# antbern/gridmap-slam-robot

Hardware: AMD Instinct MI355X
Metric: particle-scan evals/sec (higher is better)
Workload: dtype f64; 1 GPU; C3: 16384 particles/GPU x 720 beams (697 hits), 2048x2048 grid @ 0.02 m, full scan step (score+normalise+resample+ray-cast+likelihood rebuild; the rebuild is dirty-tile / factor-table-only: bit-identical results, likelihoodData on demand -- the reference's own every-cell rebuild is cpu_baseline.gpu_like_for_like_ms_per_step); particles_total=16384, particles_per_gpu=16384, beams=720, maps=1, maps_total=1, parallelism=single GPU, inputs=resident in HBM

## Files before the change

gridmap_slam_robot_amd/csrc/gms_fused_kernels.hip:

```cpp
#include "gms_map_kernels.hip"
#include "gms_pf_kernels.hip"
#include "gms_slam_kernels.hip"

#ifndef GMS_APPLY_BLOCKS_RIDING
#define GMS_APPLY_BLOCKS_RIDING 512
#endif

#ifndef RCF_RAYS
#define RCF_RAYS 4
#endif

template <bool LOGNORM>
__global__ void __launch_bounds__(256)
k_norm_raycast(const gms_beam *__restrict__ beams, const double *__restrict__ partials, int64_t nblk_global, int32_t B,
               int32_t nw_max, uint32_t n_ray_blocks, uint32_t n_norm_blocks, uint32_t n_near_blocks, int32_t n,
               double *__restrict__ w, const float *__restrict__ pose, int64_t offset, uint32_t *__restrict__ cnt,
               int32_t *__restrict__ bbox, PackedParticle *__restrict__ packed, double *__restrict__ cum,
               double *__restrict__ chunk_tot, int64_t nchunks, double *__restrict__ p2, PfStatsDev *__restrict__ stats,
               double *__restrict__ logd, uint32_t *__restrict__ cnt_pend, const int32_t *__restrict__ bbox_pend,
               const double *__restrict__ logw_lognorm, uint32_t *__restrict__ res_ticket, double *__restrict__ res_pre, GridDev g) {
    extern __shared__ __align__(16) unsigned char smem[];
    GMS_STAMP(GMS_STAMP_ROW(2, blockIdx.x), 0);
    if (blockIdx.x >= n_ray_blocks + n_norm_blocks) {
        apply_body(g, logd, cnt_pend, bbox_pend, nullptr, blockIdx.x - n_ray_blocks - n_norm_blocks, 0,
                   gridDim.x - n_ray_blocks - n_norm_blocks);
        GMS_STAMP(GMS_STAMP_ROW(2, blockIdx.x), 15);
        return;
    }
    if (blockIdx.x < n_ray_blocks) {
        __shared__ RedLds L;
        const bool near = blockIdx.x >= n_ray_blocks - n_near_blocks;
        const RayPre pre = near ? raycast_near_prologue(beams, B, B, blockIdx.x - (n_ray_blocks - n_near_blocks), 0, smem)
                                : raycast_prologue<RCF_RAYS, 4>(beams, B, B, nullptr, nw_max, blockIdx.x, 0, smem);
        const int cols[4] = { COL_SUM, COL_XW, COL_YW, COL_TW };
        double f[4];
        if (LOGNORM) {
            fold_lognorm<4>(partials, nblk_global, cols, f, L);
        } else {
            fold_sums<4>(partials, nblk_global, cols, f, L);
        }
        const float wpose[3] = { (float)(f[1] / f[0]), (float)(f[2] / f[0]), (float)(f[3] / f[0]) };
        GMS_STAMP(GMS_STAMP_ROW(2, blockIdx.x), 1);
        if (near) raycast_near_body(g, pre, wpose, cnt, bbox, 0, smem);
        else raycast_body<false, RCF_RAYS, 4>(g, pre, wpose, B, nullptr, cnt, bbox, nullptr, nullptr, 0, nullptr, blockIdx.x, 0, smem, n_near_blocks ? 1 : 0);
    } else {
        normalize_pack_body(partials, nblk_global, w, pose, n, offset, packed, cum, chunk_tot, nchunks, p2, stats,
                            blockIdx.x - n_ray_blocks, 0, LOGNORM ? logw_lognorm : (const double *)nullptr, res_ticket, n_norm_blocks,
                            res_pre, smem);
        GMS_STAMP(GMS_STAMP_ROW(2, blockIdx.x), 14);
    }
}

__global__ void __launch_bounds__(256)
k_partials_apply(const double *__restrict__ part, const float *__restrict__ pose, PfStatsDev *__restrict__ lognorm_stats, int32_t n,
                 int32_t part_nseg, int64_t offset, int64_t nblk_global, double *__restrict__ w, double *__restrict__ logw,
                 double *__restrict__ partials, double *__restrict__ logd, uint32_t *__restrict__ cnt,
                 const int32_t *__restrict__ bbox, int32_t *__restrict__ bbox_idle, GridDev g) {
    if (blockIdx.x < (uint32_t)nblk_global)
        partials_body(w, logw, pose, n, offset, nblk_global, partials, part, part_nseg, blockIdx.x, blockIdx.y, lognorm_stats);
    else
        apply_body(g, logd, cnt, bbox, bbox_idle, blockIdx.x - (uint32_t)nblk_global, blockIdx.y, gridDim.x - (uint32_t)nblk_global);
}

__global__ void __launch_bounds__(256)
k_partials_pack_apply(const double *__restrict__ part, const float *__restrict__ pose, int32_t n, int32_t part_nseg,
                      uint32_t n_local_blocks, int64_t offset, int64_t nblk_global, double *__restrict__ w, double *__restrict__ logw,
                      double *__restrict__ partials, PackedParticle *__restrict__ packed_local, double *__restrict__ logd,
                      uint32_t *__restrict__ cnt, const int32_t *__restrict__ bbox, int32_t *__restrict__ bbox_idle, GridDev g) {
    if (blockIdx.x < n_local_blocks) {
// ... 58 lines not shown
        likelihood_body<KH, SPLIT>(g, logd, lik, fac, fac_stride, taps_g, bbox, 1, tiles_x, tiles_y, blockIdx.x - n_res_blocks,
                                   blockIdx.y, gridDim.x - n_res_blocks, smem, cnt_pending, tile_state, lik_mode);
    GMS_STAMP(GMS_STAMP_ROW(3, blockIdx.x), blockIdx.x < n_res_blocks ? 1 : 2);
}

__global__ void __launch_bounds__(256)
k_deskew_motion(const double *__restrict__ angle, const double *__restrict__ distance, const uint8_t *__restrict__ hit, int32_t length,
                double d_center, double d_theta, gms_beam *__restrict__ beams_out, uint32_t n_deskew_blocks,
                float *__restrict__ pose, float *__restrict__ cs, int32_t n, int64_t offset, double d_center_sd, double d_theta_sd,
                uint64_t seed, uint64_t sequence) {
    if (blockIdx.x < n_deskew_blocks)
        deskew_body(angle, distance, hit, length, d_center, d_theta, beams_out, (int32_t)(blockIdx.x * 256u + threadIdx.x));
    else
        motion_body(pose, cs, n, offset, d_center, d_theta, d_center_sd, d_theta_sd, seed, sequence, 0,
                    (int32_t)((blockIdx.x - n_deskew_blocks) * 256u + threadIdx.x));
}

bool gms_can_pair_launches(const gms_pf *pf, int32_t B) {
    const gms_map *m = pf->map;
    return pf->n_maps == 1 && B > 0 && B <= GMS_MAX_BEAMS && !m->need_full_build && m->pair_launches;
}

void gms_launch_norm_raycast(gms_pf *pf, const double *d_partials, PackedParticle *d_packed_local, bool own,
                             const gms_beam *d_beams, int32_t B) {
    gms_map *m = pf->map;
    ProfScope ps(m, GMS_K_RAYCAST);
    const uint32_t n_near = rc_near_blocks(m, B);
    const uint32_t n_ray = (uint32_t)((B + RCF_RAYS - 1) / RCF_RAYS) + n_near, n_norm = (uint32_t)((pf->n + 255) / 256);
    const int64_t nch = nchunks_of(pf);
    const size_t smem_pre = own ? (size_t)(nch + 1 + (nch + 63) / 64 + 1) * sizeof(double) : 0;
    size_t smem = rc_smem(m, RCF_RAYS, n_near);
    if (smem < smem_pre) smem = smem_pre;
    const uint32_t n_apply = m->apply_pending ? apply_blocks(m, GMS_APPLY_BLOCKS_RIDING) : 0u;
    int32_t *pend = map_box(m);
    int32_t *bb = n_apply ? map_box(m, true) : pend;
    auto launch = [&](auto lognorm) {
        gms_launch<k_norm_raycast<lognorm()>>(m, dim3(n_ray + n_norm + n_apply), dim3(256), smem, d_beams, d_partials, nblk_global_of(pf), B,
                                              rc_nw_max(m), n_ray, n_norm, n_near, pf->n, pf->d_w, pf->d_pose, pf->offset, m->d_cnt, bb, d_packed_local,
                                              own ? pf->d_cum : (double *)nullptr, own ? pf->d_chunk_tot : (double *)nullptr, nchunks_of(pf),
                                              own ? pf->d_p2 : (double *)nullptr, pf->d_stats, m->d_log, m->d_cnt_pend, pend,
                                              lognorm() ? (const double *)pf->d_logw : (const double *)nullptr,
                                              own ? pf->d_res_ticket : (uint32_t *)nullptr, pf->d_res_pre, m->gd);
    };
    if (gms_pf_lognorm_now(pf)) launch(gms_c<true>{}); else launch(gms_c<false>{});
    if (n_apply) gms_apply_done(m);
    pf_normalized(pf, own, own);
}

void gms_launch_partials_apply(gms_pf *pf, double *d_partials, bool apply_rides_later) {
    gms_map *m = pf->map;
    if (!m->apply_pending || apply_rides_later) { gms_launch_pf_partials(pf, d_partials); return; }
    ProfScope ps(m, GMS_K_REDUCE);
    const int64_t nblk = nblk_global_of(pf);
    const uint32_t n_apply = apply_blocks(m, GMS_APPLY_BLOCKS);
    PfStatsDev *lognorm_stats = gms_pf_lognorm_now(pf) ? pf->d_stats : (PfStatsDev *)nullptr;
    hipLaunchKernelGGL(k_partials_apply, dim3((uint32_t)nblk + n_apply, pf->n_maps), dim3(256), 0, m->stream,
                       pf->pending_nseg ? (const double *)pf->d_part : (const double *)nullptr, pf->d_pose, lognorm_stats, pf->n,
                       pf->pending_nseg, pf->offset, nblk, pf->d_w, pf->d_logw, d_partials, m->d_log, m->d_cnt_pend,
                       map_box(m), map_box(m, true), m->gd);
    pf_weights_combined(pf);
    gms_apply_done(m);
}

void gms_launch_lik_resample(gms_pf *pf, double fraction) {
    gms_map *m = pf->map;
    gms_launch_pf_chunk_sums(pf);
    const double *pre = pf->res_pre_ready ? (const double *)pf->d_res_pre : (const double *)nullptr;
// ... 68 lines not shown
```

gridmap_slam_robot_amd/csrc/gms_host.hip:

```cpp
#include <math.h>
#include <dlfcn.h>
#include <stdarg.h>
#include <stddef.h>
#include <stdio.h>
#include <stdlib.h>
#include <string.h>

#include <new>
#include <algorithm>
#include <vector>

#include "gms_internal.h"

static thread_local char g_err[512] = "";

int gms_fail(int code, const char *fmt, ...) {
    va_list ap;
    va_start(ap, fmt);
    vsnprintf(g_err, sizeof(g_err), fmt, ap);
    va_end(ap);
    return code;
}

static int32_t j_d2i_host(double d) {
// ... 829 lines not shown
    HIPCHK(hipSetDevice(m->device));
    return gms_set_stamp_buffer(m, dev_buffer) ? GMS_OK : gms_fail(GMS_ERR_STATE, "this build carries no stage stamps (compile with -DGMS_STAMPS)");
}

int gms_debug_f32(gms_map *m, int32_t op, const float *in, float *out, int64_t n) {
    REQUIRE(m && in && out && n > 0 && op >= 0 && op <= 5 && (op != 3 || n % 64 == 0), "gms_debug_f32: bad arguments");
    HIPCHK(hipSetDevice(m->device));
    float *d_a = nullptr, *d_o = nullptr;
    HIPCHK(hipMalloc(&d_a, n * sizeof(float)));
    HIPCHK(hipMalloc(&d_o, n * sizeof(float)));
    HIPCHK(hipMemcpyAsync(d_a, in, n * sizeof(float), hipMemcpyHostToDevice, m->stream));
    gms_launch_debug_f32(m, op, d_a, d_o, n);
    HIPCHK(hipMemcpyAsync(out, d_o, n * sizeof(float), hipMemcpyDeviceToHost, m->stream));
    HIPCHK(hipStreamSynchronize(m->stream));
    hipFree(d_a); hipFree(d_o);
    return GMS_OK;
}

static int64_t nblk_of(int64_t n) { return (n + GMS_BLOCK - 1) / GMS_BLOCK; }
static int64_t nchunks_of(int64_t n) { return (n + 63) / 64; }

static void pf_free_global(gms_pf *pf) {
    hipFree(pf->d_partials); hipFree(pf->d_p2); hipFree(pf->d_global_own); hipFree(pf->d_chunk_tot); hipFree(pf->d_cum);
    hipFree(pf->d_res_pre); hipFree(pf->d_res_ticket);
    pf->d_partials = pf->d_p2 = nullptr; pf->d_global = pf->d_global_own = nullptr; pf->d_chunk_tot = pf->d_cum = nullptr;
    pf->d_res_pre = nullptr; pf->d_res_ticket = nullptr; pf->res_pre_ready = 0; pf->have_global = 0;
}

static int pf_alloc_global(gms_pf *pf) {
    pf_free_global(pf);
    const size_t M = pf->n_maps;
    const size_t nblk = nblk_of(pf->n_global), nch = nchunks_of(pf->n_global);
    HIPCHK(hipMalloc(&pf->d_partials, M * nblk * GMS_PARTIAL_STRIDE * sizeof(double)));
    HIPCHK(hipMalloc(&pf->d_p2, M * nblk * 2 * sizeof(double)));
    HIPCHK(hipMalloc(&pf->d_global_own, M * pf->n_global * sizeof(PackedParticle)));
    pf->d_global = pf->d_global_own;
    HIPCHK(hipMalloc(&pf->d_chunk_tot, M * (nch + 1 + nch * 8) * sizeof(double)));
    HIPCHK(hipMalloc(&pf->d_cum, M * pf->n_global * sizeof(double)));
    HIPCHK(hipMalloc(&pf->d_res_pre, M * (nch + 3) * sizeof(double)));
    HIPCHK(hipMalloc(&pf->d_res_ticket, M * sizeof(uint32_t)));
    HIPCHK(hipMemsetAsync(pf->d_res_ticket, 0, M * sizeof(uint32_t), pf->map->stream));
    return GMS_OK;
}

int gms_pf_destroy(gms_pf *pf) {
    if (!pf) return GMS_OK;
    hipSetDevice(pf->map->device);
    hipStreamSynchronize(pf->map->stream);
    pf->map->n_filters--;
    hipFree(pf->d_pose); hipFree(pf->d_pose2); hipFree(pf->d_part); hipFree(pf->d_cs2);
    hipFree(pf->d_w); hipFree(pf->d_w2); hipFree(pf->d_logw); hipFree(pf->d_cs); hipFree(pf->d_hitbeams);
    hipFree(pf->d_nhit); hipFree(pf->d_stats); hipFree(pf->d_r01); hipFree(pf->d_idx);
    hipFree(pf->d_ord); hipFree(pf->d_perm);
    hipFree(pf->modes.d_part); hipFree(pf->modes.d_bins); hipFree(pf->modes.d_table); hipFree(pf->modes.d_ctl);
    if (pf->modes.h_ctl) hipHostFree(pf->modes.h_ctl);
    hipFree(pf->beam.d_tab); ring_free(pf->beam.ring);
// ... 382 lines not shown
                        double resample_fraction, int32_t integrate) {
    return slam_update_impl(pf, dev_xytheta, nullptr, dev_beams, B, B, r01, resample_fraction, integrate);
}

int gms_slam_update_u_dev(gms_pf *pf, double d_center, double d_theta, uint64_t seed, uint64_t sequence, const gms_beam *dev_beams,
                          int32_t B, const double *r01, double resample_fraction, int32_t integrate) {
    MotionModel mo;
    mo.d_center = d_center; mo.d_theta = d_theta; mo.seed = seed; mo.sequence = sequence;
    return slam_update_impl(pf, nullptr, &mo, dev_beams, B, B, r01, resample_fraction, integrate);
}

static int slam_update_impl(gms_pf *pf, const float *dev_xytheta, const MotionModel *motion, const gms_beam *dev_beams, int32_t B,
                            int32_t beam_stride, const double *r01, double resample_fraction, int32_t integrate) {
    REQUIRE(pf && dev_beams && r01, "null argument");
    int rc = refuse_owned_maps(pf);
    if (rc) return rc;
    gms_map *m = pf->map;
    if (pf_is_shard(pf))
        return gms_fail(GMS_ERR_STATE, "sharded filter: the collectives belong to the caller (see distributed.py)");
    const ScanIn at_pose = dev_scan(dev_beams, B, beam_stride, nullptr, pf, 0);
    rc = set_poses_and_score_dev(pf, dev_xytheta, dev_beams, B, beam_stride, pf->refine != 0, motion);
    const bool pair = !rc && integrate && !pf->reference_order && beam_stride == B;
    if (pair && gms_can_pair_launches(pf, B)) {
        gms_launch_partials_apply(pf, pf->d_partials, true);
        gms_launch_norm_raycast(pf, pf->d_partials, pf->d_global_own, true, dev_beams, B);
        return paired_likelihood_resample(pf, r01, resample_fraction);
    }
    if (pair && pf->n_maps > 1 && B > 0 && !m->need_full_build && m->pair_launches) {
        const bool ride = gms_raycast_tiled(m, B);
        gms_launch_partials_apply(pf, pf->d_partials, ride);
        gms_launch_pf_apply_partials(pf, pf->d_partials, pf->d_global_own, true);
        ScanDev d;
        scan_pose(m, at_pose, &d);
        gms_launch_raycast(m, dev_beams, B, B, d.poses, d.pose_stride, ride);
        return paired_likelihood_resample(pf, r01, resample_fraction);
    }
    if (!rc) rc = gms_pf_normalize(pf, nullptr);
    if (!rc && resample_fraction >= 0.0) rc = gms_pf_resample_if(pf, r01, resample_fraction);
    if (!rc && integrate) rc = map_scan(m, at_pose, SCAN_UPDATE_MAY_DEFER);
    return rc;
}

int gms_slam_frame(gms_pf *pf, const double *angle, const double *distance, const uint8_t *hit, int32_t length, double d_center,
                   double d_theta, uint64_t seed, uint64_t sequence, const double *r01, double resample_fraction, int32_t integrate) {
    REQUIRE(pf && angle && distance && hit && r01, "null argument");
    gms_map *m = pf->map;
    if (pf->n_maps != 1) return gms_fail(GMS_ERR_STATE, "gms_slam_frame: one map per handle (a frame is one robot's revolution)");
    if (pf_is_shard(pf))
// ... 509 lines not shown
```

gridmap_slam_robot_amd/csrc/gms_internal.h:

```cpp
#pragma once

#include <hip/hip_runtime.h>
#include <stdint.h>

#include <atomic>
#include <mutex>
#include <type_traits>
#include <vector>

#include "gridmapslam.h"

struct GridDev {
    int32_t W, H;
    int64_t cells;
    double posx, posy;
    double res;
    double rinv;
    float resf;
    double l_free, l_occ;
    int32_t extra;
    float half_tol;
    double z_hit;
    double c_rand;
    double inv_max;
// ... 176 lines not shown
    m->fac_current = 1;
    m->need_full_build = 0;
}
static inline void map_box_consumed(gms_map *m) {
    if (m->bbox_dirty) { m->bbox_cur = 1 - m->bbox_cur; m->bbox_dirty = 0; }
}

struct gms_pf {
    gms_map *map;
    int32_t n;
    int64_t offset;
    int64_t n_global;
    int32_t n_maps;
    float *d_pose;
    float *d_pose2;
    float *d_cs2;
    double *d_w, *d_w2;
    double *d_logw, *d_logw2;
    float *d_cs;
    double *d_hitbeams;
    double *d_part;
    int32_t *d_nhit;
    double *d_partials;
    double *d_p2;
    PackedParticle *d_global_own;
    double *d_chunk_tot;
    double *d_cum;
    double *d_res_pre;
    uint32_t *d_res_ticket;
    PfStatsDev *d_stats;
    PfStatsDev *h_stats;
    double *d_r01;
    const double *d_r01_src;
    double r01_scalar;
    int32_t *d_idx;
    float *h_stage;
    StageRing pose_ring;
    StageRing r01_ring;
    int32_t refine;
    float4 *d_ord;
    int32_t *d_perm;
    int32_t log_norm;
    int32_t score_threads;
    int32_t reference_order;
    int32_t score_spread;
    int32_t order_mode;
// ... 308 lines not shown
    void fetch(void *dst, size_t part, size_t bytes) { out[n_out].dst = dst; out[n_out].part = part; out[n_out++].bytes = bytes; }
    int finish(int32_t *shown);
};
struct QuerySource {
    gms_map *m;
    gms_slam *s;
    int32_t index, filter;
};
static inline QuerySource query_map(gms_map *m, int32_t mi) { return {m, nullptr, mi, 0}; }
static inline QuerySource query_slam(gms_slam *s, int32_t which) { return {s ? s->map : nullptr, s, which, 0}; }
int query_check(QuerySource &src, const char *what, const char *filter_name);
int query_plane(const QuerySource &src, int32_t mode, int32_t *d_shown, uint32_t *d_dst, const uint32_t **plane);
int gms_clear_launch(gms_map *m, const uint32_t *d_plane, const gms_clearance *c, uint16_t *d_out);
int gms_reach_inflate(gms_map *m, const uint32_t *d_obstacles, int32_t inflate, int32_t mode, const uint32_t **d_blocked);

void gms_launch_pf_init(gms_pf *pf);
void gms_launch_pf_pose_trig(gms_pf *pf, const float *d_src);
void gms_launch_pf_combine(gms_pf *pf);
void gms_launch_pf_motion(gms_pf *pf, double d_center, double d_theta, uint64_t seed, uint64_t sequence);
void gms_launch_pf_chunk_sums(gms_pf *pf);
void gms_launch_partials_apply(gms_pf *pf, double *d_partials, bool apply_rides_later = false);
bool gms_can_pair_launches(const gms_pf *pf, int32_t B);
void gms_launch_norm_raycast(gms_pf *pf, const double *d_partials, PackedParticle *d_packed_local, bool own,
                             const gms_beam *d_beams, int32_t B);
void gms_launch_lik_resample(gms_pf *pf, double fraction);
void gms_launch_deskew_motion(gms_pf *pf, const double *d_angle, const double *d_distance, const uint8_t *d_hit, int32_t length,
                              double d_center, double d_theta, uint64_t seed, uint64_t sequence);
void gms_launch_partials_pack_apply(gms_pf *pf, bool apply_rides_later = false);
void gms_launch_raycast_norm_chunks(gms_pf *pf, const gms_beam *d_beams, int32_t B, bool raycast);
void gms_launch_pf_fold_neff(gms_pf *pf);
struct MotionModel {
    double d_center, d_theta;
    uint64_t seed, sequence;
};
static inline void motion_deviations(double d_center, double d_theta, double *d_center_sd, double *d_theta_sd) {
    *d_center_sd = (0.01 + fabs(d_center) * 0.05) / 2;
    *d_theta_sd = 5 * (3.141592653589793 / 180.0) + 0.1 * fabs(d_theta);
}
void gms_launch_pf_score(gms_pf *pf, const gms_beam *d_beams, int32_t B, int32_t beam_stride, const float *d_pose_src = nullptr,
                         const MotionModel *motion = nullptr);
void gms_launch_pf_partials(gms_pf *pf, double *d_partials);
bool gms_pf_lognorm_now(const gms_pf *pf);
void gms_launch_pf_pack(gms_pf *pf, PackedParticle *d_packed);
void gms_launch_pf_apply_partials(gms_pf *pf, const double *d_partials, PackedParticle *d_packed_local, bool own);
void gms_launch_pf_stats_only(gms_pf *pf, const double *d_partials, PfStatsDev *d_stats_out);
void gms_launch_pf_resample(gms_pf *pf, double fraction );
void gms_launch_pf_refine(gms_pf *pf, const gms_beam *d_beams, int32_t B, int32_t beam_stride);
void gms_launch_pf_normalize_seq(gms_pf *pf, PfStatsDev *d_stats_out, bool normalise);
void gms_launch_pf_resample_seq(gms_pf *pf, double fraction);
SlamBufs gms_slam_bufs(const gms_slam *s);
void gms_launch_slam_likelihood(gms_map *m, const SlamBufs &sb, int32_t n);
void gms_launch_slam_deskew(gms_map *m, const double *angle, const double *distance, const uint8_t *hit, int32_t L, int32_t S, int32_t Lmax,
                            int32_t length, double d_center, double d_theta, const SlamFilterArgs *tab_src, SlamFilterArgs *tab_dst, gms_beam *d_out,
                            int32_t out_pitch);
void gms_launch_slam_particle(gms_pf *pf, const gms_beam *d_beams, int32_t B, const SlamBufs &sb, bool field_in_memory, const MotionModel *motion,
                              int32_t integrate, int64_t code_words, const SlamBatch *batch = nullptr);
void gms_launch_slam_likelihood_codes(gms_map *m, const SlamBufs &sb, int64_t code_words, int32_t n, int32_t plane);
void gms_launch_slam_codes_from_log(gms_map *m, const SlamBufs &sb, int32_t first, int32_t count, int64_t code_words);
int64_t gms_slam_code_words(int64_t cells);
void gms_launch_slam_trace(gms_pf *pf, const gms_beam *d_beams, int32_t B, int32_t particle, int32_t *d_cells, uint8_t *d_cls, int32_t cap, int32_t *d_counts);
bool gms_launch_slam_refine(gms_pf *pf, const gms_beam *d_beams, int32_t B, const SlamBufs &sb, const MotionModel *motion, int32_t field_in_lds,
                            int64_t code_words, const SlamBatch *batch = nullptr);
bool gms_slam_refine_from_planes(const gms_map *m, int32_t B, int32_t field_in_lds, int64_t code_words);
int gms_align_check_for(const gms_align_params *p, const char *who);
bool gms_slam_align_from_planes(const gms_slam *s, int32_t B);
// ... 42 lines not shown
```

gridmap_slam_robot_amd/csrc/gms_pf_kernels.hip:

```cpp
#include "gms_device.h"
#include "gms_slam_device.h"

#define SCAN_CHUNK 64
#define RES_SUB_MAX_CHUNKS 1024

__global__ void k_pf_init(float *pose, float *cs, double *w, double *logw, int64_t total, double w0) {
    int64_t i = (int64_t)blockIdx.x * blockDim.x + threadIdx.x;
    if (i < total) {
        pose[3 * i] = 0.0f; pose[3 * i + 1] = 0.0f; pose[3 * i + 2] = 0.0f;
        cs[2 * i] = 1.0f; cs[2 * i + 1] = 0.0f;
        w[i] = w0; logw[i] = 0.0;
    }
}

__global__ void __launch_bounds__(256)
k_pose_trig(const float *__restrict__ src, float *__restrict__ dst, float *__restrict__ cs, int64_t total) {
    const int64_t i = (int64_t)blockIdx.x * blockDim.x + threadIdx.x;
    if (i >= total) return;
    const float x = src[3 * i], y = src[3 * i + 1], th = src[3 * i + 2];
    dst[3 * i] = x; dst[3 * i + 1] = y; dst[3 * i + 2] = th;
    float c, s;
    pose_trig(th, c, s);
    cs[2 * i] = c; cs[2 * i + 1] = s;
}
// ... 425 lines not shown
    const int32_t wave = threadIdx.x >> 6, g4 = (wave >> 2) << 2;
    GMS_STAMP(GMS_STAMP_ROW(1, blockIdx.x), 3);
    __syncthreads();
    if ((threadIdx.x & 63) == 0) {
#pragma unroll
        for (int c = 0; c < 6; c++) L.m[c][wave] = sums[c];
        L.m[6][wave] = mv; L.m[7][wave] = mx; L.m[8][wave] = ml;
    }
    __syncthreads();
    GMS_STAMP(GMS_STAMP_ROW(1, blockIdx.x), 4);
#pragma unroll
    for (int c = 0; c < 6; c++) sums[c] = ((L.m[c][g4] + L.m[c][g4 + 1]) + L.m[c][g4 + 2]) + L.m[c][g4 + 3];
    mv = L.m[6][g4]; mx = L.m[7][g4]; ml = L.m[8][g4];
    for (int k = 1; k < 4; k++) {
        argmax_merge(mv, mx, L.m[6][g4 + k], L.m[7][g4 + k]);
        if (L.m[8][g4 + k] > ml) ml = L.m[8][g4 + k];
    }
    (void)mli;
    out[COL_SUM] = sums[0]; out[COL_NZ] = sums[1]; out[COL_SQ] = sums[2];
    out[COL_XW] = sums[3]; out[COL_YW] = sums[4]; out[COL_TW] = sums[5];
    out[COL_MAX] = mv; out[COL_ARG] = mx; out[COL_MLW] = ml;
}

__device__ __forceinline__ double fold_sum(const double *__restrict__ p, int64_t nblk, int col, double *lds) {
    double acc = 0.0;
    for (int64_t b = threadIdx.x & (GRP - 1); b < nblk; b += GRP) acc += p[b * GMS_PARTIAL_STRIDE + col];
    return group_sum(acc, lds);
}

template <int NC>
__device__ __forceinline__ void fold_sums(const double *__restrict__ p, int64_t nblk, const int (&col)[NC], double (&out)[NC],
                                          RedLds &L) {
    static_assert(NC <= GMS_PARTIAL_STRIDE, "RedLds::m has GMS_PARTIAL_STRIDE rows");
    double acc[NC];
#pragma unroll
    for (int c = 0; c < NC; c++) acc[c] = 0.0;
    for (int64_t b = threadIdx.x & (GRP - 1); b < nblk; b += GRP) {
        double v[NC];
#pragma unroll
        for (int c = 0; c < NC; c++) v[c] = p[b * GMS_PARTIAL_STRIDE + col[c]];
#pragma unroll
        for (int c = 0; c < NC; c++) acc[c] += v[c];
    }
#pragma unroll
    for (int c = 0; c < NC; c++) acc[c] = wave_sum_f64(acc[c]);
    const int32_t wave = threadIdx.x >> 6, g4 = (wave >> 2) << 2;
    __syncthreads();
    if ((threadIdx.x & 63) == 0) {
#pragma unroll
        for (int c = 0; c < NC; c++) L.m[c][wave] = acc[c];
    }
    __syncthreads();
#pragma unroll
    for (int c = 0; c < NC; c++) out[c] = ((L.m[c][g4] + L.m[c][g4 + 1]) + L.m[c][g4 + 2]) + L.m[c][g4 + 3];
}

template <int NC>
__device__ __forceinline__ void fold_sums_scaled(const double *__restrict__ p, int64_t nblk, const int (&col)[NC], double (&out)[NC],
                                                 RedLds &L, double M) {
    static_assert(NC <= GMS_PARTIAL_STRIDE, "RedLds::m has GMS_PARTIAL_STRIDE rows");
    const double R = lognorm_ref(M);
    double acc[NC];
#pragma unroll
    for (int c = 0; c < NC; c++) acc[c] = 0.0;
    for (int64_t b = threadIdx.x & (GRP - 1); b < nblk; b += GRP) {
        double v[NC];
#pragma unroll
        for (int c = 0; c < NC; c++) v[c] = p[b * GMS_PARTIAL_STRIDE + col[c]];
        const double sc = exp(lognorm_ref(p[b * GMS_PARTIAL_STRIDE + COL_MLW]) - R);
#pragma unroll
        for (int c = 0; c < NC; c++) acc[c] += v[c] * sc;
    }
#pragma unroll
    for (int c = 0; c < NC; c++) acc[c] = wave_sum_f64(acc[c]);
    const int32_t wave = threadIdx.x >> 6, g4 = (wave >> 2) << 2;
    __syncthreads();
    if ((threadIdx.x & 63) == 0) {
#pragma unroll
        for (int c = 0; c < NC; c++) L.m[c][wave] = acc[c];
    }
    __syncthreads();
#pragma unroll
    for (int c = 0; c < NC; c++) out[c] = ((L.m[c][g4] + L.m[c][g4 + 1]) + L.m[c][g4 + 2]) + L.m[c][g4 + 3];
}

__device__ __forceinline__ void fold_argmax(const double *__restrict__ p, int64_t nblk, int colv, int coli, double &mv,
                                            double &mx, RedLds &L);
template <int NC>
__device__ __forceinline__ double fold_lognorm(const double *__restrict__ p, int64_t nblk, const int (&col)[NC], double (&out)[NC], RedLds &L) {
    if (nblk > GRP) {
        double ml, mli;
        fold_argmax(p, nblk, COL_MLW, -1, ml, mli, L);
        fold_sums_scaled<NC>(p, nblk, col, out, L, ml);
        return ml;
    }
    const int64_t b = threadIdx.x & (GRP - 1);
    const bool in = b < nblk;
    double v[NC];
#pragma unroll
    for (int c = 0; c < NC; c++) v[c] = in ? p[b * GMS_PARTIAL_STRIDE + col[c]] : 0.0;
    const double mb = in ? p[b * GMS_PARTIAL_STRIDE + COL_MLW] : -INFINITY;
    double mloc = mb == mb ? mb : -INFINITY;
#define GMS_STEP_(O) { const double v2 = wave_xor<O>(mloc); if (v2 > mloc) mloc = v2; }
    GMS_BUTTERFLY(GMS_STEP_)
#undef GMS_STEP_
    const int32_t wave = threadIdx.x >> 6, g4 = (wave >> 2) << 2;
    __syncthreads();
    if ((threadIdx.x & 63) == 0) L.b[wave] = mloc;
    __syncthreads();
    double M = L.b[g4];
    for (int k = 1; k < 4; k++) if (L.b[g4 + k] > M) M = L.b[g4 + k];
    const double sc = in ? exp(lognorm_ref(mb) - lognorm_ref(M)) : 0.0;
    double acc[NC];
#pragma unroll
    for (int c = 0; c < NC; c++) acc[c] = wave_sum_f64(0.0 + v[c] * sc);
    if ((threadIdx.x & 63) == 0) {
#pragma unroll
        for (int c = 0; c < NC; c++) L.m[c][wave] = acc[c];
    }
    __syncthreads();
#pragma unroll
    for (int c = 0; c < NC; c++) out[c] = ((L.m[c][g4] + L.m[c][g4 + 1]) + L.m[c][g4 + 2]) + L.m[c][g4 + 3];
    return M;
}

__device__ __forceinline__ void fold_argmax(const double *__restrict__ p, int64_t nblk, int colv, int coli, double &mv,
                                            double &mx, RedLds &L) {
    mv = -INFINITY; mx = 9.0e15;
    bool first = true;
    for (int64_t b = threadIdx.x & (GRP - 1); b < nblk; b += GRP) {
        const double v2 = p[b * GMS_PARTIAL_STRIDE + colv], i2 = coli >= 0 ? p[b * GMS_PARTIAL_STRIDE + coli] : (double)b;
        if (first) { mv = v2; mx = i2; first = false; } else argmax_merge(mv, mx, v2, i2);
    }
    group_argmax(mv, mx, L.a, L.b);
}

__device__ __forceinline__ double fold_stats(const double *__restrict__ p, int64_t nblk, PfStatsDev *s, bool write,
                                             const float *__restrict__ pose, int64_t pose_base, int64_t pose_n, RedLds &L,
                                             const PackedParticle *__restrict__ glob = nullptr, bool lognorm = false, double *ref_out = nullptr) {
    double ml = 0.0, mli;
    if (!write) {
        if (!lognorm) return fold_sum(p, nblk, COL_SUM, L.a);
        const int c1[1] = { COL_SUM };
        double f1[1];
        ml = fold_lognorm<1>(p, nblk, c1, f1, L);
        if (ref_out) *ref_out = ml;
        return f1[0];
    }
    const int cols[5] = { COL_SUM, COL_NZ, COL_XW, COL_YW, COL_TW };
    double f[5];
    if (lognorm) { ml = fold_lognorm<5>(p, nblk, cols, f, L); if (ref_out) *ref_out = ml; }
    else fold_sums<5>(p, nblk, cols, f, L);
    const double sum = f[0], nz = f[1], xw = f[2], yw = f[3], tw = f[4];
    double mv, mx;
    fold_argmax(p, nblk, COL_MAX, COL_ARG, mv, mx, L);
    if (!lognorm) fold_argmax(p, nblk, COL_MLW, -1, ml, mli, L);
    if (threadIdx.x == 0) {
        s->n_ambiguous = 0;
        s->weight_sum = sum;
        s->max_w = lognorm ? exp(ml - lognorm_ref(ml)) : mv;
        s->strongest = mx < 8.0e15 ? (int32_t)mx : 0;
        if (!lognorm) s->n_zero = (int32_t)nz;
        s->max_logw = ml;
        s->xs = xw; s->ys = yw; s->ts = tw;
        s->wpose[0] = (float)(xw / sum);
        s->wpose[1] = (float)(yw / sum);
        s->wpose[2] = (float)(tw / sum);
        const int64_t st = (int64_t)s->strongest - pose_base;
        if (glob) {
            const PackedParticle pp = glob[s->strongest];
            s->spose[0] = pp.x; s->spose[1] = pp.y; s->spose[2] = pp.theta;
        } else if (pose && st >= 0 && st < pose_n) {
            s->spose[0] = pose[3 * st]; s->spose[1] = pose[3 * st + 1]; s->spose[2] = pose[3 * st + 2];
        }
    }
    return sum;
}

__device__ __forceinline__ int64_t block_count(int64_t n, int64_t blk) {
// ... 32 lines not shown
    const int64_t nlb = ((int64_t)n + GMS_BLOCK - 1) / GMS_BLOCK;
    double *p = partials + ((size_t)mi * nblk_global + gb) * GMS_PARTIAL_STRIDE;
    if (lb < 0 || lb >= nlb) {
        if (threadIdx.x < GMS_PARTIAL_STRIDE) p[threadIdx.x] = 0.0;
        return;
    }
    double out[GMS_PARTIAL_STRIDE];
    const size_t o = (size_t)mi * n + lb * GMS_BLOCK;
    block_partials(w + o, logw + o, pose + 3 * o, block_count(n, lb), offset + lb * GMS_BLOCK, out, L, part, mi, n,
                   part_nseg, lb * GMS_BLOCK, lognorm_stats != nullptr);
    if (threadIdx.x == 0)
        for (int k = 0; k < GMS_PARTIAL_STRIDE; k++) p[k] = out[k];
}

__global__ void __launch_bounds__(256)
k_partials(const double *__restrict__ part, const float *__restrict__ pose, PfStatsDev *__restrict__ lognorm_stats, int32_t n,
           int32_t part_nseg, int64_t offset, int64_t nblk_global, double *__restrict__ w, double *__restrict__ logw,
           double *__restrict__ partials) {
    GMS_STAMP(GMS_STAMP_ROW(1, blockIdx.x), 0);
    partials_body(w, logw, pose, n, offset, nblk_global, partials, part, part_nseg, blockIdx.x, blockIdx.y, lognorm_stats);
    GMS_STAMP(GMS_STAMP_ROW(1, blockIdx.x), 1);
}

__device__ __forceinline__ double *chunk_sub_of(double *chunk_tot_all, int64_t nchunks, int32_t n_maps, int32_t mi) {
    return chunk_tot_all + (size_t)n_maps * (nchunks + 1) + (size_t)mi * nchunks * 8;
}
__device__ __forceinline__ void block_chunk_scan(double v, int64_t i, int64_t n_pop, int64_t blk, int64_t nchunks,
                                                 double *__restrict__ cum, double *__restrict__ chunk_tot,
                                                 double *__restrict__ p2_blk, double *__restrict__ sub, bool through = false) {
    __shared__ double s_ct[4][2];
    const int32_t lane = threadIdx.x & 63, wave = threadIdx.x >> 6;
    double inc = v;
#pragma unroll
    for (int o = 1; o < 64; o <<= 1) {
        const double up = __shfl_up(inc, o, GMS_WAVE);
        if (lane >= o) inc += up;
    }
    const double sq = wave_sum_f64(v * v);
    const double tot = __shfl(inc, 63, GMS_WAVE);
    if (i < n_pop) cum[i] = inc;
    if ((lane & 7) == 7 && blk * 4 + wave < nchunks) sub[(blk * 4 + wave) * 8 + (lane >> 3)] = inc;
    if (lane == 0) {
        const int64_t c = blk * 4 + wave;
        if (c < nchunks) { if (through) store_through(&chunk_tot[c], tot); else chunk_tot[c] = tot; }
        s_ct[wave][0] = tot; s_ct[wave][1] = sq;
    }
// ... 66 lines not shown
    double tv[8];
#pragma unroll
    for (int k = 0; k < 8; k++) { const int64_t c = (int64_t)threadIdx.x + k * (int64_t)blockDim.x; tv[k] = c < nchunks ? load_coherent<true>(&tot[c]) : 0.0; }
    double norm_sum, sq_sum;
    fold_neff<true>(p2, nblk, norm_sum, sq_sum, lds);
#pragma unroll
    for (int k = 0; k < 8; k++) { const int64_t c = (int64_t)threadIdx.x + k * (int64_t)blockDim.x; if (c < nchunks) off[c] = tv[k]; }
    for (int64_t c0 = (int64_t)threadIdx.x + 8 * (int64_t)blockDim.x; c0 < nchunks; c0 += 8 * (int64_t)blockDim.x) {
        double v[8];
#pragma unroll
        for (int k = 0; k < 8; k++) { const int64_t c = c0 + k * (int64_t)blockDim.x; v[k] = c < nchunks ? load_coherent<true>(&tot[c]) : 0.0; }
#pragma unroll
        for (int k = 0; k < 8; k++) { const int64_t c = c0 + k * (int64_t)blockDim.x; if (c < nchunks) off[c] = v[k]; }
    }
    chunk_offsets_scan(off, nchunks);
    for (int64_t c = threadIdx.x; c <= nchunks; c += blockDim.x) pre[c] = off[c];
    if (threadIdx.x == 0) {
        pre[nchunks + 1] = norm_sum; pre[nchunks + 2] = sq_sum;
        stats->norm_sum = norm_sum; stats->sq_sum = sq_sum;
    }
    GMS_STAMP(GMS_STAMP_ROW(2, blockIdx.x), 13);
}

__device__ __forceinline__ void
normalize_pack_body(const double *__restrict__ partials_all, int64_t nblk_global, double *__restrict__ w,
                    const float *__restrict__ pose, int32_t n, int64_t offset, PackedParticle *__restrict__ packed,
                    double *__restrict__ cum, double *__restrict__ chunk_tot, int64_t nchunks,
                    double *__restrict__ p2_all, PfStatsDev *__restrict__ stats, uint32_t bx, uint32_t by,
                    const double *__restrict__ logw_lognorm = nullptr, uint32_t *__restrict__ ticket = nullptr,
                    uint32_t n_blocks = 0, double *__restrict__ pre = nullptr, unsigned char *smem = nullptr) {
    __shared__ RedLds L;
    const int32_t mi = (int32_t)by;
    const double *p = partials_all + (size_t)mi * nblk_global * GMS_PARTIAL_STRIDE;
    double M = 0.0;
    const double sum = fold_stats(p, nblk_global, stats + mi, bx == 0, pose + (size_t)mi * n * 3, offset, n, L, nullptr, logw_lognorm != nullptr, &M);
    const int32_t i = (int32_t)bx * 256 + threadIdx.x;
    double wn = 0.0;
    if (logw_lognorm) {
        const double v = i < n ? exp(logw_lognorm[(size_t)mi * n + i] - lognorm_ref(M)) : 1.0;
        const int32_t zeros = __popcll(__ballot(v == 0.0));
        if ((threadIdx.x & 63) == 0 && zeros) atomicAdd(&stats[mi].n_zero, zeros);
        if (i < n) w[(size_t)mi * n + i] = v;
    }
    if (i < n) {
        const size_t gi = (size_t)mi * n + i;
        wn = w[gi] / sum;
        w[gi] = wn;
        PackedParticle pp;
        pp.w = wn; pp.x = pose[3 * gi]; pp.y = pose[3 * gi + 1]; pp.theta = pose[3 * gi + 2]; pp.pad = 0u;
        packed[gi] = pp;
    }
    if (cum)
        block_chunk_scan(wn, i, n, bx, nchunks, cum + (size_t)mi * n, chunk_tot + (size_t)mi * (nchunks + 1),
                         p2_all + ((size_t)mi * nblk_global + bx) * 2, chunk_sub_of(chunk_tot, nchunks, (int32_t)gridDim.y, mi),
                         ticket != nullptr);
    if (cum && ticket) resample_prefix_last(p2_all + (size_t)mi * nblk_global * 2, nblk_global, chunk_tot + (size_t)mi * (nchunks + 1),
                                            nchunks, ticket + mi, n_blocks, pre + (size_t)mi * (nchunks + 3), stats + mi, smem, L.a);
}
// ... 532 lines not shown

void gms_launch_pf_combine(gms_pf *pf) {
    if (!pf->pending_nseg) return;
    gms_map *m = pf->map;
    ProfScope ps(m, GMS_K_SCORE);
    hipLaunchKernelGGL(k_score_combine, dim3((pf->n + 255) / 256, pf->n_maps), dim3(256), 0, m->stream, pf->d_part, pf->n,
                       pf->pending_nseg, pf->d_w, pf->d_logw);
    pf_weights_combined(pf);
}

bool gms_pf_lognorm_now(const gms_pf *pf) { return pf->log_norm && pf->score_fresh; }

void gms_launch_pf_partials(gms_pf *pf, double *d_partials) {
    gms_map *m = pf->map;
    ProfScope ps(m, GMS_K_REDUCE);
    const int64_t nblk = nblk_global_of(pf);
    hipLaunchKernelGGL(k_partials, dim3((unsigned)nblk, pf->n_maps), dim3(256), 0, m->stream,
                       pf->pending_nseg ? (const double *)pf->d_part : (const double *)nullptr, pf->d_pose,
                       gms_pf_lognorm_now(pf) ? pf->d_stats : (PfStatsDev *)nullptr, pf->n, pf->pending_nseg, pf->offset, nblk,
                       pf->d_w, pf->d_logw, d_partials);
    pf_weights_combined(pf);
}

void gms_launch_pf_apply_partials(gms_pf *pf, const double *d_partials, PackedParticle *d_packed_local, bool own) {
    gms_map *m = pf->map;
    ProfScope ps(m, GMS_K_REDUCE);
    const int64_t nblk = nblk_global_of(pf);
    hipLaunchKernelGGL(k_normalize_pack, dim3((pf->n + 255) / 256, pf->n_maps), dim3(256), 0, m->stream, d_partials, nblk,
                       pf->d_w, pf->d_pose, pf->n, pf->offset, d_packed_local, own ? pf->d_cum : (double *)nullptr,
                       own ? pf->d_chunk_tot : (double *)nullptr, nchunks_of(pf), own ? pf->d_p2 : (double *)nullptr, pf->d_stats,
                       gms_pf_lognorm_now(pf) ? (const double *)pf->d_logw : (const double *)nullptr);
    pf_normalized(pf, own, false);
}

void gms_launch_pf_stats_only(gms_pf *pf, const double *d_partials, PfStatsDev *d_stats_out) {
    gms_map *m = pf->map;
    ProfScope ps(m, GMS_K_REDUCE);
    hipLaunchKernelGGL(k_stats_only, dim3(pf->n_maps), dim3(256), 0, m->stream, d_partials, nblk_global_of(pf), pf->d_pose,
                       pf->n, pf->offset, d_stats_out);
}

void gms_launch_pf_pack(gms_pf *pf, PackedParticle *d_packed) {
    gms_map *m = pf->map;
    hipLaunchKernelGGL(k_pack, dim3((pf->n + 255) / 256, pf->n_maps), dim3(256), 0, m->stream, pf->d_w, pf->d_pose,
                       pf->n, d_packed);
    if (d_packed == pf->d_global) pf_source_written(pf, 0);
// ... 54 lines not shown
```

Measured before the change: 386.4 million particle-scan evals/s.

## Compute particle-weight partials per wavefront instead of per 256-thread block

Adds a k_partials_wave kernel with one 64-lane wavefront per block. Each block writes one partial-statistics row per wavefront and skips the LDS/cross-wave block reduction. The downstream folds (fold_sums, fold_argmax, fold_stats) gain a WAVE mode that reads four wave rows per former block row and sums them in fixed order, so the results stay bit-identical. The path applies only to single-map, non-lognorm, non-sharded runs. When the partials-apply fusion is not used, any pending map apply rides along in the norm_raycast launch instead. The cost is four times as many partial rows to read in the fold and many tiny 64-thread blocks.

```diff
diff --git a/gridmap_slam_robot_amd/csrc/gms_fused_kernels.hip b/gridmap_slam_robot_amd/csrc/gms_fused_kernels.hip
--- a/gridmap_slam_robot_amd/csrc/gms_fused_kernels.hip
+++ b/gridmap_slam_robot_amd/csrc/gms_fused_kernels.hip
@@ -10,7 +10,7 @@
 #define RCF_RAYS 4
 #endif
 
-template <bool LOGNORM>
+template <bool LOGNORM, bool WAVE>
 __global__ void __launch_bounds__(256)
 k_norm_raycast(const gms_beam *__restrict__ beams, const double *__restrict__ partials, int64_t nblk_global, int32_t B,
                int32_t nw_max, uint32_t n_ray_blocks, uint32_t n_norm_blocks, uint32_t n_near_blocks, int32_t n,
@@ -20,6 +20,7 @@
                double *__restrict__ logd, uint32_t *__restrict__ cnt_pend, const int32_t *__restrict__ bbox_pend,
                const double *__restrict__ logw_lognorm, uint32_t *__restrict__ res_ticket, double *__restrict__ res_pre, GridDev g) {
     extern __shared__ __align__(16) unsigned char smem[];
+    static_assert(!(LOGNORM && WAVE), "a log-normalising pass needs its block's reference: block rows");
     GMS_STAMP(GMS_STAMP_ROW(2, blockIdx.x), 0);
     if (blockIdx.x >= n_ray_blocks + n_norm_blocks) {
         apply_body(g, logd, cnt_pend, bbox_pend, nullptr, blockIdx.x - n_ray_blocks - n_norm_blocks, 0,
@@ -37,14 +38,14 @@
         if (LOGNORM) {
             fold_lognorm<4>(partials, nblk_global, cols, f, L);
         } else {
-            fold_sums<4>(partials, nblk_global, cols, f, L);
+            fold_sums<4, WAVE>(partials, nblk_global, cols, f, L, ((int64_t)n + 63) / 64);
         }
         const float wpose[3] = { (float)(f[1] / f[0]), (float)(f[2] / f[0]), (float)(f[3] / f[0]) };
         GMS_STAMP(GMS_STAMP_ROW(2, blockIdx.x), 1);
         if (near) raycast_near_body(g, pre, wpose, cnt, bbox, 0, smem);
         else raycast_body<false, RCF_RAYS, 4>(g, pre, wpose, B, nullptr, cnt, bbox, nullptr, nullptr, 0, nullptr, blockIdx.x, 0, smem, n_near_blocks ? 1 : 0);
     } else {
-        normalize_pack_body(partials, nblk_global, w, pose, n, offset, packed, cum, chunk_tot, nchunks, p2, stats,
+        normalize_pack_body<WAVE>(partials, nblk_global, w, pose, n, offset, packed, cum, chunk_tot, nchunks, p2, stats,
                             blockIdx.x - n_ray_blocks, 0, LOGNORM ? logw_lognorm : (const double *)nullptr, res_ticket, n_norm_blocks,
                             res_pre, smem);
         GMS_STAMP(GMS_STAMP_ROW(2, blockIdx.x), 14);
@@ -149,7 +150,7 @@
 }
 
 void gms_launch_norm_raycast(gms_pf *pf, const double *d_partials, PackedParticle *d_packed_local, bool own,
-                             const gms_beam *d_beams, int32_t B) {
+                             const gms_beam *d_beams, int32_t B, bool wave_rows) {
     gms_map *m = pf->map;
     ProfScope ps(m, GMS_K_RAYCAST);
     const uint32_t n_near = rc_near_blocks(m, B);
@@ -161,15 +162,17 @@
     const uint32_t n_apply = m->apply_pending ? apply_blocks(m, GMS_APPLY_BLOCKS_RIDING) : 0u;
     int32_t *pend = map_box(m);
     int32_t *bb = n_apply ? map_box(m, true) : pend;
-    auto launch = [&](auto lognorm) {
-        gms_launch<k_norm_raycast<lognorm()>>(m, dim3(n_ray + n_norm + n_apply), dim3(256), smem, d_beams, d_partials, nblk_global_of(pf), B,
+    auto launch = [&](auto lognorm, auto wave) {
+        gms_launch<k_norm_raycast<lognorm(), wave()>>(m, dim3(n_ray + n_norm + n_apply), dim3(256), smem, d_beams, d_partials, nblk_global_of(pf), B,
                                               rc_nw_max(m), n_ray, n_norm, n_near, pf->n, pf->d_w, pf->d_pose, pf->offset, m->d_cnt, bb, d_packed_local,
                                               own ? pf->d_cum : (double *)nullptr, own ? pf->d_chunk_tot : (double *)nullptr, nchunks_of(pf),
                                               own ? pf->d_p2 : (double *)nullptr, pf->d_stats, m->d_log, m->d_cnt_pend, pend,
                                               lognorm() ? (const double *)pf->d_logw : (const double *)nullptr,
                                               own ? pf->d_res_ticket : (uint32_t *)nullptr, pf->d_res_pre, m->gd);
     };
-    if (gms_pf_lognorm_now(pf)) launch(gms_c<true>{}); else launch(gms_c<false>{});
+    if (gms_pf_lognorm_now(pf)) launch(gms_c<true>{}, gms_c<false>{});
+    else if (wave_rows) launch(gms_c<false>{}, gms_c<true>{});
+    else launch(gms_c<false>{}, gms_c<false>{});
     if (n_apply) gms_apply_done(m);
     pf_normalized(pf, own, own);
 }
diff --git a/gridmap_slam_robot_amd/csrc/gms_host.hip b/gridmap_slam_robot_amd/csrc/gms_host.hip
--- a/gridmap_slam_robot_amd/csrc/gms_host.hip
+++ b/gridmap_slam_robot_amd/csrc/gms_host.hip
@@ -875,8 +875,8 @@
 
 static void pf_free_global(gms_pf *pf) {
     hipFree(pf->d_partials); hipFree(pf->d_p2); hipFree(pf->d_global_own); hipFree(pf->d_chunk_tot); hipFree(pf->d_cum);
-    hipFree(pf->d_res_pre); hipFree(pf->d_res_ticket);
-    pf->d_partials = pf->d_p2 = nullptr; pf->d_global = pf->d_global_own = nullptr; pf->d_chunk_tot = pf->d_cum = nullptr;
+    hipFree(pf->d_res_pre); hipFree(pf->d_res_ticket); hipFree(pf->d_wave_partials);
+    pf->d_partials = pf->d_p2 = pf->d_wave_partials = nullptr; pf->d_global = pf->d_global_own = nullptr; pf->d_chunk_tot = pf->d_cum = nullptr;
     pf->d_res_pre = nullptr; pf->d_res_ticket = nullptr; pf->res_pre_ready = 0; pf->have_global = 0;
 }
 
@@ -885,6 +885,7 @@
     const size_t M = pf->n_maps;
     const size_t nblk = nblk_of(pf->n_global), nch = nchunks_of(pf->n_global);
     HIPCHK(hipMalloc(&pf->d_partials, M * nblk * GMS_PARTIAL_STRIDE * sizeof(double)));
+    HIPCHK(hipMalloc(&pf->d_wave_partials, nch * GMS_PARTIAL_STRIDE * sizeof(double)));
     HIPCHK(hipMalloc(&pf->d_p2, M * nblk * 2 * sizeof(double)));
     HIPCHK(hipMalloc(&pf->d_global_own, M * pf->n_global * sizeof(PackedParticle)));
     pf->d_global = pf->d_global_own;
@@ -1313,8 +1314,10 @@
     rc = set_poses_and_score_dev(pf, dev_xytheta, dev_beams, B, beam_stride, pf->refine != 0, motion);
     const bool pair = !rc && integrate && !pf->reference_order && beam_stride == B;
     if (pair && gms_can_pair_launches(pf, B)) {
-        gms_launch_partials_apply(pf, pf->d_partials, true);
-        gms_launch_norm_raycast(pf, pf->d_partials, pf->d_global_own, true, dev_beams, B);
+        const bool wave_rows = gms_pf_wave_partials_now(pf);
+        if (wave_rows) gms_launch_pf_partials_wave(pf);
+        else gms_launch_partials_apply(pf, pf->d_partials, true);
+        gms_launch_norm_raycast(pf, wave_rows ? pf->d_wave_partials : pf->d_partials, pf->d_global_own, true, dev_beams, B, wave_rows);
         return paired_likelihood_resample(pf, r01, resample_fraction);
     }
     if (pair && pf->n_maps > 1 && B > 0 && !m->need_full_build && m->pair_launches) {
diff --git a/gridmap_slam_robot_amd/csrc/gms_internal.h b/gridmap_slam_robot_amd/csrc/gms_internal.h
--- a/gridmap_slam_robot_amd/csrc/gms_internal.h
+++ b/gridmap_slam_robot_amd/csrc/gms_internal.h
@@ -222,6 +222,7 @@
     double *d_part;
     int32_t *d_nhit;
     double *d_partials;
+    double *d_wave_partials;
     double *d_p2;
     PackedParticle *d_global_own;
     double *d_chunk_tot;
@@ -576,7 +577,7 @@
 void gms_launch_partials_apply(gms_pf *pf, double *d_partials, bool apply_rides_later = false);
 bool gms_can_pair_launches(const gms_pf *pf, int32_t B);
 void gms_launch_norm_raycast(gms_pf *pf, const double *d_partials, PackedParticle *d_packed_local, bool own,
-                             const gms_beam *d_beams, int32_t B);
+                             const gms_beam *d_beams, int32_t B, bool wave_rows = false);
 void gms_launch_lik_resample(gms_pf *pf, double fraction);
 void gms_launch_deskew_motion(gms_pf *pf, const double *d_angle, const double *d_distance, const uint8_t *d_hit, int32_t length,
                               double d_center, double d_theta, uint64_t seed, uint64_t sequence);
@@ -595,6 +596,8 @@
                          const MotionModel *motion = nullptr);
 void gms_launch_pf_partials(gms_pf *pf, double *d_partials);
 bool gms_pf_lognorm_now(const gms_pf *pf);
+bool gms_pf_wave_partials_now(const gms_pf *pf);
+void gms_launch_pf_partials_wave(gms_pf *pf);
 void gms_launch_pf_pack(gms_pf *pf, PackedParticle *d_packed);
 void gms_launch_pf_apply_partials(gms_pf *pf, const double *d_partials, PackedParticle *d_packed_local, bool own);
 void gms_launch_pf_stats_only(gms_pf *pf, const double *d_partials, PfStatsDev *d_stats_out);
diff --git a/gridmap_slam_robot_amd/csrc/gms_pf_kernels.hip b/gridmap_slam_robot_amd/csrc/gms_pf_kernels.hip
--- a/gridmap_slam_robot_amd/csrc/gms_pf_kernels.hip
+++ b/gridmap_slam_robot_amd/csrc/gms_pf_kernels.hip
@@ -471,23 +471,102 @@
     out[COL_MAX] = mv; out[COL_ARG] = mx; out[COL_MLW] = ml;
 }
 
-__device__ __forceinline__ double fold_sum(const double *__restrict__ p, int64_t nblk, int col, double *lds) {
+__device__ __forceinline__ void wave_partials(double *__restrict__ w, double *__restrict__ logw, const float *__restrict__ pose,
+                                              int32_t n, int64_t i, double out[GMS_PARTIAL_STRIDE],
+                                              const double *__restrict__ part, int32_t part_nseg) {
+    const bool in = i < n;
+    double v, lw;
+    if (part) {
+        v = 0.0; lw = -INFINITY;
+        if (in) {
+            combine_segments(part, 0, n, part_nseg, i, v, lw);
+            w[i] = v; logw[i] = lw;
+        }
+    } else {
+        v = in ? w[i] : 0.0;
+        lw = in ? logw[i] : -INFINITY;
+    }
+    const float px = in ? pose[3 * i] : 0.0f, py = in ? pose[3 * i + 1] : 0.0f, pt = in ? pose[3 * i + 2] : 0.0f;
+    double s = 0.0, nz = 0.0, mv = -INFINITY, mx = 9.0e15, ml = -INFINITY, sq = 0.0, xw = 0.0, yw = 0.0, tw = 0.0;
+    if (in) {
+        s += v;
+        sq += v * v;
+        xw += (double)px * v;
+        yw += (double)py * v;
+        tw += angle_constrain((double)pt) * v;
+        if (v == 0.0) nz += 1.0;
+        if (v > mv) { mv = v; mx = (double)i; }
+        else if (mx > 8.0e15 && v == v) { mv = v; mx = (double)i; }
+        if (lw > ml) ml = lw;
+    }
+    GMS_STAMP(GMS_STAMP_ROW(1, blockIdx.x), 2);
+    double sums[6] = { s, nz, sq, xw, yw, tw };
+#pragma unroll
+    for (int c = 0; c < 6; c++) sums[c] = wave_sum_f64(sums[c]);
+#define GMS_STEP_(O) { const double v2 = wave_xor<O>(mv), i2 = wave_xor<O>(mx); argmax_merge(mv, mx, v2, i2); \
+                       const double l2 = wave_xor<O>(ml); if (l2 > ml) ml = l2; }
+    GMS_BUTTERFLY(GMS_STEP_)
+#undef GMS_STEP_
+    GMS_STAMP(GMS_STAMP_ROW(1, blockIdx.x), 3);
+    out[COL_SUM] = sums[0]; out[COL_NZ] = sums[1]; out[COL_SQ] = sums[2];
+    out[COL_XW] = sums[3]; out[COL_YW] = sums[4]; out[COL_TW] = sums[5];
+    out[COL_MAX] = mv; out[COL_ARG] = mx; out[COL_MLW] = ml;
+}
+
+__device__ __forceinline__ void wave_rows_load(const double *__restrict__ p, int64_t b, int col, int64_t nwaves, double missing,
+                                               double (&r)[4]) {
+#pragma unroll
+    for (int k = 0; k < 4; k++) {
+        const int64_t wv = 4 * b + k;
+        const double v = p[(wv < nwaves ? wv : nwaves - 1) * GMS_PARTIAL_STRIDE + col];
+        r[k] = wv < nwaves ? v : missing;
+    }
+}
+__device__ __forceinline__ double wave_rows_sum(const double (&r)[4]) { return ((r[0] + r[1]) + r[2]) + r[3]; }
+__device__ __forceinline__ double wave_rows_max(const double (&r)[4]) {
+    double m = r[0];
+    for (int k = 1; k < 4; k++) if (r[k] > m) m = r[k];
+    return m;
+}
+__device__ __forceinline__ void wave_rows_argmax(const double (&rv)[4], const double (&ri)[4], double &v, double &i) {
+    v = rv[0]; i = ri[0];
+    for (int k = 1; k < 4; k++) argmax_merge(v, i, rv[k], ri[k]);
+}
+
+template <bool WAVE = false>
+__device__ __forceinline__ double fold_sum(const double *__restrict__ p, int64_t nblk, int col, double *lds, int64_t nwaves = 0) {
     double acc = 0.0;
-    for (int64_t b = threadIdx.x & (GRP - 1); b < nblk; b += GRP) acc += p[b * GMS_PARTIAL_STRIDE + col];
+    for (int64_t b = threadIdx.x & (GRP - 1); b < nblk; b += GRP) {
+        if constexpr (WAVE) {
+            double r[4];
+            wave_rows_load(p, b, col, nwaves, 0.0, r);
+            acc += wave_rows_sum(r);
+        } else {
+            acc += p[b * GMS_PARTIAL_STRIDE + col];
+        }
+    }
     return group_sum(acc, lds);
 }
 
-template <int NC>
+template <int NC, bool WAVE = false>
 __device__ __forceinline__ void fold_sums(const double *__restrict__ p, int64_t nblk, const int (&col)[NC], double (&out)[NC],
-                                          RedLds &L) {
+                                          RedLds &L, int64_t nwaves = 0) {
     static_assert(NC <= GMS_PARTIAL_STRIDE, "RedLds::m has GMS_PARTIAL_STRIDE rows");
     double acc[NC];
 #pragma unroll
     for (int c = 0; c < NC; c++) acc[c] = 0.0;
     for (int64_t b = threadIdx.x & (GRP - 1); b < nblk; b += GRP) {
         double v[NC];
-#pragma unroll
-        for (int c = 0; c < NC; c++) v[c] = p[b * GMS_PARTIAL_STRIDE + col[c]];
+        if constexpr (WAVE) {
+            double r[NC][4];
+#pragma unroll
+            for (int c = 0; c < NC; c++) wave_rows_load(p, b, col[c], nwaves, 0.0, r[c]);
+#pragma unroll
+            for (int c = 0; c < NC; c++) v[c] = wave_rows_sum(r[c]);
+        } else {
+#pragma unroll
+            for (int c = 0; c < NC; c++) v[c] = p[b * GMS_PARTIAL_STRIDE + col[c]];
+        }
 #pragma unroll
         for (int c = 0; c < NC; c++) acc[c] += v[c];
     }
@@ -533,8 +612,9 @@
     for (int c = 0; c < NC; c++) out[c] = ((L.m[c][g4] + L.m[c][g4 + 1]) + L.m[c][g4 + 2]) + L.m[c][g4 + 3];
 }
 
+template <bool WAVE = false>
 __device__ __forceinline__ void fold_argmax(const double *__restrict__ p, int64_t nblk, int colv, int coli, double &mv,
-                                            double &mx, RedLds &L);
+                                            double &mx, RedLds &L, int64_t nwaves = 0);
 template <int NC>
 __device__ __forceinline__ double fold_lognorm(const double *__restrict__ p, int64_t nblk, const int (&col)[NC], double (&out)[NC], RedLds &L) {
     if (nblk > GRP) {
@@ -573,23 +653,39 @@
     return M;
 }
 
+template <bool WAVE>
 __device__ __forceinline__ void fold_argmax(const double *__restrict__ p, int64_t nblk, int colv, int coli, double &mv,
-                                            double &mx, RedLds &L) {
+                                            double &mx, RedLds &L, int64_t nwaves) {
     mv = -INFINITY; mx = 9.0e15;
     bool first = true;
     for (int64_t b = threadIdx.x & (GRP - 1); b < nblk; b += GRP) {
-        const double v2 = p[b * GMS_PARTIAL_STRIDE + colv], i2 = coli >= 0 ? p[b * GMS_PARTIAL_STRIDE + coli] : (double)b;
+        double v2, i2;
+        if constexpr (WAVE) {
+            double rv[4], ri[4];
+            wave_rows_load(p, b, colv, nwaves, -INFINITY, rv);
+            if (coli >= 0) {
+                wave_rows_load(p, b, coli, nwaves, 9.0e15, ri);
+                wave_rows_argmax(rv, ri, v2, i2);
+            } else {
+                v2 = wave_rows_max(rv); i2 = (double)b;
+            }
+        } else {
+            v2 = p[b * GMS_PARTIAL_STRIDE + colv]; i2 = coli >= 0 ? p[b * GMS_PARTIAL_STRIDE + coli] : (double)b;
+        }
         if (first) { mv = v2; mx = i2; first = false; } else argmax_merge(mv, mx, v2, i2);
     }
     group_argmax(mv, mx, L.a, L.b);
 }
 
+template <bool WAVE = false>
 __device__ __forceinline__ double fold_stats(const double *__restrict__ p, int64_t nblk, PfStatsDev *s, bool write,
                                              const float *__restrict__ pose, int64_t pose_base, int64_t pose_n, RedLds &L,
-                                             const PackedParticle *__restrict__ glob = nullptr, bool lognorm = false, double *ref_out = nullptr) {
+                                             const PackedParticle *__restrict__ glob = nullptr, bool lognorm = false, double *ref_out = nullptr,
+                                             int64_t nwaves = 0) {
     double ml = 0.0, mli;
+    if constexpr (WAVE) lognorm = false;
     if (!write) {
-        if (!lognorm) return fold_sum(p, nblk, COL_SUM, L.a);
+        if (!lognorm) return fold_sum<WAVE>(p, nblk, COL_SUM, L.a, nwaves);
         const int c1[1] = { COL_SUM };
         double f1[1];
         ml = fold_lognorm<1>(p, nblk, c1, f1, L);
@@ -599,11 +695,11 @@
     const int cols[5] = { COL_SUM, COL_NZ, COL_XW, COL_YW, COL_TW };
     double f[5];
     if (lognorm) { ml = fold_lognorm<5>(p, nblk, cols, f, L); if (ref_out) *ref_out = ml; }
-    else fold_sums<5>(p, nblk, cols, f, L);
+    else fold_sums<5, WAVE>(p, nblk, cols, f, L, nwaves);
     const double sum = f[0], nz = f[1], xw = f[2], yw = f[3], tw = f[4];
     double mv, mx;
-    fold_argmax(p, nblk, COL_MAX, COL_ARG, mv, mx, L);
-    if (!lognorm) fold_argmax(p, nblk, COL_MLW, -1, ml, mli, L);
+    fold_argmax<WAVE>(p, nblk, COL_MAX, COL_ARG, mv, mx, L, nwaves);
+    if (!lognorm) fold_argmax<WAVE>(p, nblk, COL_MLW, -1, ml, mli, L, nwaves);
     if (threadIdx.x == 0) {
         s->n_ambiguous = 0;
         s->weight_sum = sum;
@@ -682,6 +778,31 @@
     GMS_STAMP(GMS_STAMP_ROW(1, blockIdx.x), 1);
 }
 
+#ifndef GMS_WAVE_PARTIALS_XCD_BLOCKS
+#define GMS_WAVE_PARTIALS_XCD_BLOCKS 0
+#endif
+static_assert(EPT == 1 && GMS_BLOCK == 4 * GMS_WAVE, "a reduction block is four wavefronts of one particle per lane");
+__global__ void __launch_bounds__(64)
+k_partials_wave(const double *__restrict__ part, const float *__restrict__ pose, int32_t n, int32_t part_nseg,
+                double *__restrict__ w, double *__restrict__ logw, double *__restrict__ rows) {
+    GMS_STAMP(GMS_STAMP_ROW(1, blockIdx.x), 0);
+#if GMS_WAVE_PARTIALS_XCD_BLOCKS
+    const uint32_t j = blockIdx.x >> 3;
+    const int64_t wv = 4 * (int64_t)((j >> 2) * 8 + (blockIdx.x & 7)) + (j & 3);
+#else
+    const int64_t wv = blockIdx.x;
+#endif
+    if (wv * GMS_WAVE >= n) return;
+    double out[GMS_PARTIAL_STRIDE];
+    wave_partials(w, logw, pose, n, wv * GMS_WAVE + threadIdx.x, out, part, part_nseg);
+    if (threadIdx.x == 0) {
+        double *p = rows + wv * GMS_PARTIAL_STRIDE;
+#pragma unroll
+        for (int k = 0; k < GMS_PARTIAL_STRIDE; k++) p[k] = out[k];
+    }
+    GMS_STAMP(GMS_STAMP_ROW(1, blockIdx.x), 1);
+}
+
 __device__ __forceinline__ double *chunk_sub_of(double *chunk_tot_all, int64_t nchunks, int32_t n_maps, int32_t mi) {
     return chunk_tot_all + (size_t)n_maps * (nchunks + 1) + (size_t)mi * nchunks * 8;
 }
@@ -794,6 +915,7 @@
     GMS_STAMP(GMS_STAMP_ROW(2, blockIdx.x), 13);
 }
 
+template <bool WAVE = false>
 __device__ __forceinline__ void
 normalize_pack_body(const double *__restrict__ partials_all, int64_t nblk_global, double *__restrict__ w,
                     const float *__restrict__ pose, int32_t n, int64_t offset, PackedParticle *__restrict__ packed,
@@ -805,7 +927,8 @@
     const int32_t mi = (int32_t)by;
     const double *p = partials_all + (size_t)mi * nblk_global * GMS_PARTIAL_STRIDE;
     double M = 0.0;
-    const double sum = fold_stats(p, nblk_global, stats + mi, bx == 0, pose + (size_t)mi * n * 3, offset, n, L, nullptr, logw_lognorm != nullptr, &M);
+    const double sum = fold_stats<WAVE>(p, nblk_global, stats + mi, bx == 0, pose + (size_t)mi * n * 3, offset, n, L, nullptr, logw_lognorm != nullptr, &M,
+                                        ((int64_t)n + 63) / 64);
     const int32_t i = (int32_t)bx * 256 + threadIdx.x;
     double wn = 0.0;
     if (logw_lognorm) {
@@ -1384,6 +1507,23 @@
     pf_weights_combined(pf);
 }
 
+bool gms_pf_wave_partials_now(const gms_pf *pf) {
+    return pf->n_maps == 1 && pf->offset == 0 && pf->n_global == pf->n && !gms_pf_lognorm_now(pf);
+}
+
+void gms_launch_pf_partials_wave(gms_pf *pf) {
+    gms_map *m = pf->map;
+    ProfScope ps(m, GMS_K_REDUCE);
+    uint32_t grid = (uint32_t)nchunks_of(pf);
+#if GMS_WAVE_PARTIALS_XCD_BLOCKS
+    grid = (grid + 31u) / 32u * 32u;
+#endif
+    hipLaunchKernelGGL(k_partials_wave, dim3(grid), dim3(GMS_WAVE), 0, m->stream,
+                       pf->pending_nseg ? (const double *)pf->d_part : (const double *)nullptr, pf->d_pose, pf->n, pf->pending_nseg,
+                       pf->d_w, pf->d_logw, pf->d_wave_partials);
+    pf_weights_combined(pf);
+}
+
 void gms_launch_pf_apply_partials(gms_pf *pf, const double *d_partials, PackedParticle *d_packed_local, bool own) {
     gms_map *m = pf->map;
     ProfScope ps(m, GMS_K_REDUCE);
```

Measured after the change: 394.6 million particle-scan evals/s (median of 6 runs). 2.1% higher.
